# kornia/kornia

Hardware: AMD Instinct MI355X
Metric: Mpix/s fwd+bwd warp_perspective+GaussianBlur2d Bx3x512x512 (higher is better)
Workload: dtype f32; 1 GPU; configs[1]: warp_perspective bilinear + GaussianBlur2d k=5 sigma=1.5, B=256x3x512x512 fp32 fwd+bwd (grad wrt image and homography) per GPU; global_batch=256, parallelism=batch-shard x1 (weak scaling), no data-path collective

## Files before the change

kornia_amd/csrc/km_blur_fast.hip:

```cpp
#include <stdlib.h>

#include "km_regtile.h"


#ifdef KMB_ROWS_OVERRIDE
#define KMB_ROWS KMB_ROWS_OVERRIDE
#else
#define KMB_ROWS 32
#endif
#define KMB_ROWS_MID 16
#define KMB_ROWS_SMALL 8
#define KMB_FEW_WAVES_F32 4096

template <typename T>
struct KmVec4;
template <>
struct KmVec4<float> {
    typedef float4 V;
};
template <>
struct KmVec4<km_bf16> {
    typedef uint2 V;
};
template <>
struct KmVec4<km_f16> {
    typedef uint2 V;
};

__device__ __forceinline__ float km_round_store(float v, const float*) { return v; }
__device__ __forceinline__ float km_round_store(float v, const km_bf16*) { return __uint_as_float(((uint32_t)km_f32_to_bf16_bits(v)) << 16); }
__device__ __forceinline__ float km_round_store(float v, const km_f16*) { KM_OPAQUE(v); return (float)(_Float16)v; }


template <typename T>
struct KmBlurArgs {
    const T* x;
    T* y;
    const float* kx;
    const float* ky;
    int C, H, W, Bk, border;
    uint32_t groups_x;
    uint32_t bx, by;
    uint32_t nblocks;
    uint32_t reverse;
    uint32_t rows;
    uint32_t stream_out;
};

template <int K>
__device__ __forceinline__ void kmb_adjoint_taps(const float (&k)[K], int p, int n, int border, float (&w)[K]) {
    constexpr int L = (K - 1) / 2, R = K - 1 - L;
    const bool interior = (border == KM_BORDER_CIRCULAR) || (border == KM_BORDER_CONSTANT) || (p >= K - 1 && p <= n - K);
#pragma unroll
    for (int d = 0; d < K; ++d) w[d] = k[K - 1 - d];
    if (interior) return;
#pragma unroll
    for (int d = 0; d < K; ++d) {
        const int i = p - R + d;
        float acc = 0.f;
        if (i >= 0 && i < n) {
#pragma unroll
            for (int t = 0; t < K; ++t)
                if (km_border_map(i + t - L, n, border) == p) acc += k[t];
        }
        w[d] = acc;
    }
}

#ifndef KMB_BWD_WAVES
#define KMB_BWD_WAVES 1
#endif
template <typename T, int K, bool BWD, int ROWS = KMB_ROWS>
__global__ __launch_bounds__(256, (BWD ? KMB_BWD_WAVES : 1)) void km_blur_reg_kernel(const KmBlurArgs<T> a) {
    constexpr int L = (K - 1) / 2, R = K - 1 - L;
    constexpr bool COLF = BWD && sizeof(T) == 2;
    uint32_t bid = km_xcd_remap(blockIdx.x, a.nblocks, a.reverse);
    const uint32_t tbx = bid % a.bx;
    bid /= a.bx;
    const uint32_t tby = bid % a.by;
    const uint32_t bc = bid / a.by;
    const int lane = threadIdx.x & 63, wave = __builtin_amdgcn_readfirstlane((int)(threadIdx.x >> 6));
    const int gx = (int)tbx * 64 + lane;
    const int r0 = ((int)tby * 4 + wave) * ROWS;
    if (gx >= (int)a.groups_x || r0 >= a.H) return;
    const int H = a.H, W = a.W, border = a.border;
    const int c0 = gx * 4;
    const bool left = (c0 == 0), right = (c0 == W - 4);
    const T* img = a.x + (size_t)bc * H * W;
    T* out = a.y + (size_t)bc * H * W;
    const int b = (int)(bc / a.C);

    float kx[K], ky[K];
    {
        const float* px = a.kx + (size_t)(b % a.Bk) * K;
        const float* py = a.ky + (size_t)(b % a.Bk) * K;
#pragma unroll
        for (int t = 0; t < K; ++t) { kx[t] = px[t]; ky[t] = py[t]; }
    }
    float wx[4][K];
    if (BWD) {
#pragma unroll
        for (int o = 0; o < 4; ++o) kmb_adjoint_taps<K>(kx, c0 + o, W, border, wx[o]);
    }

    int offL = c0 - 4, offR = c0 + 4;
    if (left) offL = (border == KM_BORDER_CIRCULAR) ? W - 4 : c0;
    if (right) offR = (border == KM_BORDER_CIRCULAR) ? 0 : c0;

    float ring[K][4];
    float ring_e[COLF ? K : 1][COLF ? R : 1];
    const int n_rows = (r0 + ROWS <= H ? ROWS : H - r0);
    const int total = n_rows + K - 1;
    const bool e0 = (lane == 0), e63 = (lane == 63);

    float on4[4] = {0.f, 0.f, 0.f, 0.f}, en4[4] = {0.f, 0.f, 0.f, 0.f};
    int srow_n = -1;
    auto request = [&](int it) {
        const int rin = r0 + it - (BWD ? R : L);
        int sr;
        if (BWD) sr = (border == KM_BORDER_CIRCULAR) ? km_border_map(rin, H, KM_BORDER_CIRCULAR) : ((rin >= 0 && rin < H) ? rin : -1);
        else sr = km_border_map(rin, H, border);
        srow_n = sr;
        if (sr >= 0) {
            const T* rowp = img + (size_t)sr * W;
            km_ld4(rowp + c0, on4);
            if (border != KM_BORDER_CIRCULAR && (e0 || e63)) km_ld4(rowp + (e0 ? offL : offR), en4);
        }
    };
    request(0);

    for (int it0 = 0; it0 < total; it0 += K) {
#pragma unroll
        for (int kk = 0; kk < K; ++kk) {
            const int it = it0 + kk;
            if (it < total) {
                const int srow = srow_n;
                float v[12];
                float o4[4], e4[4];
#pragma unroll
                for (int q = 0; q < 4; ++q) { o4[q] = on4[q]; e4[q] = en4[q]; }
                if (it + 1 < total) request(it + 1);
                if (srow >= 0) {
                    const T* rowp = img + (size_t)srow * W;
                    float l4[4], r4[4];
                    if (border == KM_BORDER_CIRCULAR) {
                        km_ld4(rowp + offL, l4);
                        km_ld4(rowp + offR, r4);
                    } else {
#pragma unroll
                        for (int q = 0; q < 4; ++q) {
                            const float pl = km_prev64(o4[q]), nr = km_next64(o4[q]);
                            l4[q] = e0 ? e4[q] : pl;
                            r4[q] = e63 ? e4[q] : nr;
                        }
                    }
                    if (border != KM_BORDER_CIRCULAR) {
                        if (BWD || border == KM_BORDER_CONSTANT) {
                            if (left) { l4[0] = l4[1] = l4[2] = l4[3] = 0.f; }
                            if (right) { r4[0] = r4[1] = r4[2] = r4[3] = 0.f; }
                        } else if (border == KM_BORDER_REFLECT) {
                            if (left) { l4[0] = r4[0]; l4[1] = o4[3]; l4[2] = o4[2]; l4[3] = o4[1]; }
                            if (right) { const float t3 = l4[3]; r4[0] = o4[2]; r4[1] = o4[1]; r4[2] = o4[0]; r4[3] = t3; }
                        } else {
                            if (left) { l4[0] = l4[1] = l4[2] = l4[3] = o4[0]; }
                            if (right) { r4[0] = r4[1] = r4[2] = r4[3] = o4[3]; }
                        }
                    }
#pragma unroll
                    for (int q = 0; q < 4; ++q) { v[q] = l4[q]; v[4 + q] = o4[q]; v[8 + q] = r4[q]; }
                } else {
#pragma unroll
                    for (int q = 0; q < 12; ++q) v[q] = 0.f;
                }
                if constexpr (COLF) {
#pragma unroll
                    for (int o = 0; o < 4; ++o) ring[kk][o] = v[4 + o];
#pragma unroll
                    for (int j = 0; j < R; ++j) ring_e[kk][j] = e0 ? v[4 - R + j] : v[8 + j];
                } else {
#pragma unroll
                    for (int o = 0; o < 4; ++o) {
                        float acc = 0.f;
                        if (BWD) {
#pragma unroll
                            for (int d = 0; d < K; ++d) acc = km_fma(wx[o][d], v[4 + o - R + d], acc);
                        } else {
#pragma unroll
                            for (int q = 0; q < K; ++q) acc = km_fma(kx[q], v[4 + o - L + q], acc);
                        }
                        ring[kk][o] = km_round_store(acc, (const T*)nullptr);
                    }
                }
                if (it >= K - 1) {
                    const int r = r0 + it - (K - 1);
                    float res[4];
                    if constexpr (COLF) {
                        float wy[K];
                        kmb_adjoint_taps<K>(ky, r, H, border, wy);
                        float c4[4], ce[R];
#pragma unroll
                        for (int o = 0; o < 4; ++o) {
                            float acc = 0.f;
#pragma unroll
                            for (int d = 0; d < K; ++d) acc = km_fma(wy[d], ring[(kk + 1 + d) % K][o], acc);
                            c4[o] = km_round_store(acc, (const T*)nullptr);
                        }
#pragma unroll
                        for (int j = 0; j < R; ++j) {
                            float acc = 0.f;
#pragma unroll
                            for (int d = 0; d < K; ++d) acc = km_fma(wy[d], ring_e[(kk + 1 + d) % K][j], acc);
                            ce[j] = km_round_store(acc, (const T*)nullptr);
                        }
                        float u[12];
#pragma unroll
                        for (int q = 0; q < 4; ++q) {
                            const float pl = km_prev64(c4[q]), nr = km_next64(c4[q]);
                            u[q] = left ? 0.f : pl;
                            u[4 + q] = c4[q];
                            u[8 + q] = right ? 0.f : nr;
                        }
#pragma unroll
                        for (int j = 0; j < R; ++j) {
                            if (e0 && !left) u[4 - R + j] = ce[j];
                            if (e63 && !right) u[8 + j] = ce[j];
                        }
#pragma unroll
                        for (int o = 0; o < 4; ++o) {
                            float acc = 0.f;
#pragma unroll
                            for (int d = 0; d < K; ++d) acc = km_fma(wx[o][d], u[4 + o - R + d], acc);
                            res[o] = acc;
                        }
                    } else if (BWD) {
                        float wy[K];
                        kmb_adjoint_taps<K>(ky, r, H, border, wy);
#pragma unroll
                        for (int o = 0; o < 4; ++o) {
                            float acc = 0.f;
#pragma unroll
                            for (int d = 0; d < K; ++d) acc = km_fma(wy[d], ring[(kk + 1 + d) % K][o], acc);
                            res[o] = acc;
                        }
                    } else {
#pragma unroll
                        for (int o = 0; o < 4; ++o) {
                            float acc = 0.f;
#pragma unroll
                            for (int p = 0; p < K; ++p) acc = km_fma(ky[p], ring[(kk + 1 + p) % K][o], acc);
                            res[o] = acc;
                        }
                    }
                    km_st4_pol(out + (size_t)r * W + c0, res, a.stream_out != 0u);
                }
            }
        }
    }
}

template <typename T, int K, int ROWS>
static void km_blur_launch_rows(bool bwd, const KmBlurArgs<T>& a, hipStream_t s) {
    if (bwd)
        hipLaunchKernelGGL((km_blur_reg_kernel<T, K, true, ROWS>), dim3(a.nblocks), dim3(256), 0, s, a);
    else
        hipLaunchKernelGGL((km_blur_reg_kernel<T, K, false, ROWS>), dim3(a.nblocks), dim3(256), 0, s, a);
}
template <typename T, int K>
static int km_blur_launch(bool bwd, const KmBlurArgs<T>& a, hipStream_t s) {
    if (a.rows == KMB_ROWS_SMALL) km_blur_launch_rows<T, K, KMB_ROWS_SMALL>(bwd, a, s);
    else if (a.rows == KMB_ROWS_MID) km_blur_launch_rows<T, K, KMB_ROWS_MID>(bwd, a, s);
    else km_blur_launch_rows<T, K, KMB_ROWS>(bwd, a, s);
    return km_check_launch(bwd ? "km_blur_reg_bwd" : "km_blur_reg_fwd");
}

static int km_blur_rows(bool bwd, size_t elem, int K, uint64_t waves_big, int force) {
    if (force == KMB_ROWS_SMALL || force == KMB_ROWS_MID || force == KMB_ROWS) return force;
    if (elem == 2) return KMB_ROWS;
    if (waves_big < KMB_FEW_WAVES_F32 || K == 3) return KMB_ROWS_MID;
    if (K == 5) return bwd ? KMB_ROWS : KMB_ROWS_MID;
    return KMB_ROWS;
}

template <typename T>
static int km_blur_run(bool bwd, const void* x, const void* kx, const void* ky, void* y, int B, int C, int H, int W, int Bk,
                       int K, int border, hipStream_t s) {
    KmBlurArgs<T> a;
    a.x = (const T*)x; a.y = (T*)y; a.kx = (const float*)kx; a.ky = (const float*)ky;
    a.C = C; a.H = H; a.W = W; a.Bk = Bk; a.border = border;
    a.groups_x = (uint32_t)(W / 4);
    a.bx = (a.groups_x + 63) / 64;
    const int force_rows = km_config().blur_rows;
    const uint64_t waves_big = (uint64_t)a.bx * (uint64_t)((H + KMB_ROWS - 1) / KMB_ROWS) * (uint64_t)B * C;
    const int rows = km_blur_rows(bwd, sizeof(T), K, waves_big, force_rows);
    a.rows = (uint32_t)rows;
    a.by = (uint32_t)((H + 4 * rows - 1) / (4 * rows));
    const uint64_t nb = (uint64_t)a.bx * a.by * (uint64_t)B * C;
    KM_REQUIRE(nb < (1ull << 31), "km_blur: grid too large");
    a.nblocks = (uint32_t)nb;
    if (nb == 0) return 0;
    a.reverse = km_traversal_next(s);
    a.stream_out = km_stream_stores((uint64_t)B * C * H * W * sizeof(T));
    switch (K) {
        case 3: return km_blur_launch<T, 3>(bwd, a, s);
        case 5: return km_blur_launch<T, 5>(bwd, a, s);
        case 7: return km_blur_launch<T, 7>(bwd, a, s);
        default: return km_blur_launch<T, 9>(bwd, a, s);
    }
}

int km_blur_fast_supported(const void* x, const void* y, int H, int W, int kH, int kW, int border, int same, int dtype) {
    if (!same || kH != kW || (kH & 1) == 0 || kH < 3 || kH > 9) return 0;
    if (dtype == KM_F64) return 0;
    if ((W & 3) != 0 || W < 8 || H < kH) return 0;
    if (border == KM_BORDER_REFLECT && (kH - 1) / 2 >= (H < W ? H : W)) return 0;
    const size_t esz = (dtype == KM_F32) ? 4 : 2;
    if (((uintptr_t)x % (4 * esz)) != 0 || ((uintptr_t)y % (4 * esz)) != 0) return 0;
    if ((((size_t)H * W * esz) % (4 * esz)) != 0) return 0;
    return 1;
}

int km_blur_fast_bwd_supported(const void* gy, const void* gx, int H, int W, int kH, int kW, int border, int same, int dtype) {
    if (dtype != KM_F32 && border == KM_BORDER_CIRCULAR) return 0;
    return km_blur_fast_supported(gy, gx, H, W, kH, kW, border, same, dtype);
}

int km_blur_fast_run(bool bwd, const void* x, const void* kx, const void* ky, void* y, int B, int C, int H, int W, int Bk, int K,
                     int border, int dtype, hipStream_t s) {
    switch (dtype) {
        case KM_F32: return km_blur_run<float>(bwd, x, kx, ky, y, B, C, H, W, Bk, K, border, s);
        case KM_BF16: return km_blur_run<km_bf16>(bwd, x, kx, ky, y, B, C, H, W, Bk, K, border, s);
        default: return km_blur_run<km_f16>(bwd, x, kx, ky, y, B, C, H, W, Bk, K, border, s);
    }
}
```

kornia_amd/csrc/km_common.h:

```cpp
#pragma once

#include <hip/hip_runtime.h>
#include <stdint.h>

#define KM_ABI_FEATURES 3
#define KM_ABI_VERSION 3

enum { KM_F32 = 0, KM_F64 = 1, KM_BF16 = 2, KM_F16 = 3 };

void km_set_error(const char* fmt, ...);
int km_check_launch(const char* what);

#define KM_REQUIRE(cond, ...)          \
    do {                               \
        if (!(cond)) {                 \
            km_set_error(__VA_ARGS__); \
            return -1;                 \
        }                              \
    } while (0)

#ifndef KM_CHECK_ALIGNED
#define KM_CHECK_ALIGNED(p, bytes) ((void)0)
#endif

#ifndef KM_F2I
#define KM_F2I(v) ((int)(v))
#endif

#ifndef KM_CVT_RPI
__device__ __forceinline__ int km_cvt_rpi(float v) {
    int r;
    asm("v_cvt_rpi_i32_f32 %0, %1" : "=v"(r) : "v"(v));
    return r;
}
#define KM_CVT_RPI(v) km_cvt_rpi(v)
#endif

#ifndef KM_NEXT16
__device__ __forceinline__ uint32_t km_next16(uint32_t v) {
    return (uint32_t)__builtin_amdgcn_update_dpp((int)v, (int)v, 0x101, 0xf, 0xf, false);
}
__device__ __forceinline__ float km_next16(float v) { return __uint_as_float(km_next16(__float_as_uint(v))); }
__device__ __forceinline__ float km_prev16(float v) {
    return __uint_as_float((uint32_t)__builtin_amdgcn_update_dpp((int)__float_as_uint(v), (int)__float_as_uint(v), 0x111, 0xf, 0xf, false));
}
__device__ __forceinline__ uint32_t km_next64(uint32_t v) { return (uint32_t)__builtin_amdgcn_update_dpp((int)v, (int)v, 0x130, 0xf, 0xf, false); }
__device__ __forceinline__ float km_next64(float v) { return __uint_as_float(km_next64(__float_as_uint(v))); }
__device__ __forceinline__ float km_prev64(float v) {
    return __uint_as_float((uint32_t)__builtin_amdgcn_update_dpp((int)__float_as_uint(v), (int)__float_as_uint(v), 0x138, 0xf, 0xf, false));
}
__device__ __forceinline__ float km_quad_xor1(float v) {
    return __uint_as_float((uint32_t)__builtin_amdgcn_update_dpp((int)__float_as_uint(v), (int)__float_as_uint(v), 0xB1, 0xf, 0xf, false));
}
__device__ __forceinline__ float km_quad_xor2(float v) {
    return __uint_as_float((uint32_t)__builtin_amdgcn_update_dpp((int)__float_as_uint(v), (int)__float_as_uint(v), 0x4E, 0xf, 0xf, false));
}
__device__ __forceinline__ uint32_t km_wave_umax_last(uint32_t v) {
    int x = (int)v;
#define KM_UMAX_STEP(ctrl, rows) x = (int)max((uint32_t)x, (uint32_t)__builtin_amdgcn_update_dpp(x, x, ctrl, rows, 0xf, false));
    KM_UMAX_STEP(0x111, 0xf) KM_UMAX_STEP(0x112, 0xf) KM_UMAX_STEP(0x114, 0xf) KM_UMAX_STEP(0x118, 0xf)
    KM_UMAX_STEP(0x142, 0xa) KM_UMAX_STEP(0x143, 0xc)
#undef KM_UMAX_STEP
    return (uint32_t)x;
}
__device__ __forceinline__ double km_wave_sum_last(double v) {
#define KM_DSUM_STEP(ctrl, rows)                                                                                  \
    {                                                                                                             \
        const int lo_ = __builtin_amdgcn_update_dpp(0, __double2loint(v), ctrl, rows, 0xf, false);                \
        const int hi_ = __builtin_amdgcn_update_dpp(0, __double2hiint(v), ctrl, rows, 0xf, false);                \
        v += __hiloint2double(hi_, lo_);                                                                          \
    }
    KM_DSUM_STEP(0x111, 0xf) KM_DSUM_STEP(0x112, 0xf) KM_DSUM_STEP(0x114, 0xf) KM_DSUM_STEP(0x118, 0xf)
    KM_DSUM_STEP(0x142, 0xa) KM_DSUM_STEP(0x143, 0xc)
#undef KM_DSUM_STEP
    return v;
}
#endif

__device__ __forceinline__ void km_quad_transpose4(float (&a)[4], int q) {
    const bool b0 = (q & 1) != 0, b1 = (q & 2) != 0;
#pragma unroll
    for (int p = 0; p < 4; p += 2) {
        const float r = km_quad_xor1(b0 ? a[p] : a[p + 1]);
        a[p] = b0 ? r : a[p];
        a[p + 1] = b0 ? a[p + 1] : r;
    }
#pragma unroll
    for (int p = 0; p < 2; ++p) {
        const float r = km_quad_xor2(b1 ? a[p] : a[p + 2]);
        a[p] = b1 ? r : a[p];
        a[p + 2] = b1 ? a[p + 2] : r;
    }
}
template <bool STREAM>
__device__ __forceinline__ void km_st4_c(float* p, const float (&v)[4]) {
    typedef float km_f4v_ __attribute__((ext_vector_type(4)));
    km_f4v_ vv; vv.x = v[0]; vv.y = v[1]; vv.z = v[2]; vv.w = v[3];
    if constexpr (STREAM) __builtin_nontemporal_store(vv, reinterpret_cast<km_f4v_*>(p));
    else *reinterpret_cast<km_f4v_*>(p) = vv;
}

struct km_bf16 {
    uint16_t bits;
};
typedef _Float16 km_f16;

template <typename T>
struct KmTraits;
template <>
struct KmTraits<float> {
    typedef float R;
    static constexpr int code = KM_F32;
};
template <>
struct KmTraits<double> {
    typedef double R;
    static constexpr int code = KM_F64;
};
template <>
struct KmTraits<km_bf16> {
    typedef float R;
    static constexpr int code = KM_BF16;
};
template <>
struct KmTraits<km_f16> {
    typedef float R;
    static constexpr int code = KM_F16;
};

__device__ __forceinline__ float km_ld(const float* p) { return *p; }
__device__ __forceinline__ double km_ld(const double* p) { return *p; }
__device__ __forceinline__ float km_ld(const km_bf16* p) { return __uint_as_float(((uint32_t)p->bits) << 16); }
__device__ __forceinline__ float km_ld(const km_f16* p) { return (float)(*p); }

__device__ __forceinline__ uint16_t km_f32_to_bf16_bits_sw(float f) {
    uint32_t u = __float_as_uint(f);
    if ((u & 0x7fffffffu) > 0x7f800000u) return (uint16_t)((u >> 16) | 0x0040u);
    u += 0x7fffu + ((u >> 16) & 1u);
    return (uint16_t)(u >> 16);
}
#if defined(__gfx950__)
__device__ __forceinline__ uint16_t km_f32_to_bf16_bits(float f) { return __builtin_bit_cast(uint16_t, (__bf16)f); }
__device__ __forceinline__ uint32_t km_f32x2_to_bf16x2_bits(float lo, float hi) {
    typedef __bf16 km_bf2v __attribute__((ext_vector_type(2)));
    typedef float km_f2v_ __attribute__((ext_vector_type(2)));
    km_f2v_ v; v.x = lo; v.y = hi;
    return __builtin_bit_cast(uint32_t, __builtin_convertvector(v, km_bf2v));
}
#else
__device__ __forceinline__ uint16_t km_f32_to_bf16_bits(float f) { return km_f32_to_bf16_bits_sw(f); }
__device__ __forceinline__ uint32_t km_f32x2_to_bf16x2_bits(float lo, float hi) {
    return (uint32_t)km_f32_to_bf16_bits_sw(lo) | ((uint32_t)km_f32_to_bf16_bits_sw(hi) << 16);
}
#endif
#ifndef KM_OPAQUE
#define KM_OPAQUE(v) asm volatile("" : "+v"(v))
#endif
#ifndef KM_NO_NT_ST
#define KM_NT_ST 1
#endif
#ifdef KM_NT_ST
__device__ __forceinline__ void km_st(float* p, float v) { __builtin_nontemporal_store(v, p); }
#else
__device__ __forceinline__ void km_st(float* p, float v) { *p = v; }
#endif
#define KM_STREAM_MIN_BYTES (128ull << 20)
static inline uint32_t km_stream_stores(uint64_t out_bytes) {
#ifdef KM_NT_ST
    return out_bytes >= KM_STREAM_MIN_BYTES ? 1u : 0u;
#else
    (void)out_bytes;
    return 0u;
#endif
}
#ifndef KM_FWD_PLAIN_ST
#define KM_FWD_PLAIN_ST 0
#endif
template <bool STREAM>
__device__ __forceinline__ void km_st_c(float* p, float v) {
    if constexpr (STREAM && !KM_FWD_PLAIN_ST) __builtin_nontemporal_store(v, p);
    else *p = v;
}
__device__ __forceinline__ void km_st(double* p, double v) { *p = v; }
__device__ __forceinline__ void km_st(km_bf16* p, float v) { p->bits = km_f32_to_bf16_bits(v); }
__device__ __forceinline__ void km_st(km_f16* p, float v) { KM_OPAQUE(v); *p = (km_f16)v; }
template <bool STREAM>
__device__ __forceinline__ void km_st_c(double* p, double v) { *p = v; }
template <bool STREAM>
__device__ __forceinline__ void km_st_c(km_bf16* p, float v) { km_st(p, v); }
template <bool STREAM>
__device__ __forceinline__ void km_st_c(km_f16* p, float v) { km_st(p, v); }

__device__ __forceinline__ float km_round_as(float v, const float*) { return v; }
__device__ __forceinline__ double km_round_as(double v, const double*) { return v; }
__device__ __forceinline__ float km_round_as(float v, const km_bf16*) { return __uint_as_float(((uint32_t)km_f32_to_bf16_bits(v)) << 16); }
__device__ __forceinline__ float km_round_as(float v, const km_f16*) { KM_OPAQUE(v); return (float)(km_f16)v; }

struct __attribute__((packed, aligned(4))) km_f32x2_u { float x, y; };
struct __attribute__((packed, aligned(8))) km_f64x2_u { double x, y; };
struct __attribute__((packed, aligned(2))) km_u16x2_u { uint16_t x, y; };
__device__ __forceinline__ void km_ld2(const float* p, float& a, float& b) {
    const km_f32x2_u v = *reinterpret_cast<const km_f32x2_u*>(p);
    a = v.x; b = v.y;
}
__device__ __forceinline__ void km_ld2(const double* p, double& a, double& b) {
    const km_f64x2_u v = *reinterpret_cast<const km_f64x2_u*>(p);
    a = v.x; b = v.y;
}
__device__ __forceinline__ void km_ld2(const km_bf16* p, float& a, float& b) {
    const km_u16x2_u v = *reinterpret_cast<const km_u16x2_u*>(p);
    a = __uint_as_float(((uint32_t)v.x) << 16); b = __uint_as_float(((uint32_t)v.y) << 16);
}
struct __attribute__((packed, aligned(2))) km_h16x2_u { km_f16 x, y; };
__device__ __forceinline__ void km_ld2(const km_f16* p, float& a, float& b) {
    const km_h16x2_u v = *reinterpret_cast<const km_h16x2_u*>(p);
    a = (float)v.x; b = (float)v.y;
}

struct __attribute__((packed, aligned(4))) km_f32x4_u { float x, y, z, w; };
struct __attribute__((packed, aligned(8))) km_f64x4_u { double x, y, z, w; };
struct __attribute__((packed, aligned(2))) km_u16x4_u { uint16_t x, y, z, w; };
__device__ __forceinline__ void km_ld4u(const float* p, float (&o)[4]) {
    const km_f32x4_u v = *reinterpret_cast<const km_f32x4_u*>(p);
    o[0] = v.x; o[1] = v.y; o[2] = v.z; o[3] = v.w;
}
__device__ __forceinline__ void km_ld4u(const double* p, double (&o)[4]) {
    const km_f64x4_u v = *reinterpret_cast<const km_f64x4_u*>(p);
    o[0] = v.x; o[1] = v.y; o[2] = v.z; o[3] = v.w;
}
__device__ __forceinline__ void km_ld4u(const km_bf16* p, float (&o)[4]) {
    const km_u16x4_u v = *reinterpret_cast<const km_u16x4_u*>(p);
    o[0] = __uint_as_float(((uint32_t)v.x) << 16); o[1] = __uint_as_float(((uint32_t)v.y) << 16);
    o[2] = __uint_as_float(((uint32_t)v.z) << 16); o[3] = __uint_as_float(((uint32_t)v.w) << 16);
}
__device__ __forceinline__ void km_ld4u(const km_f16* p, float (&o)[4]) {
    o[0] = (float)p[0]; o[1] = (float)p[1]; o[2] = (float)p[2]; o[3] = (float)p[3];
}

template <typename T>
__device__ __forceinline__ const T* km_at(const T* base, uint32_t elem_off) {
    return reinterpret_cast<const T*>(reinterpret_cast<const char*>(base) + elem_off * (uint32_t)sizeof(T));
}

template <typename T>
__device__ __forceinline__ T* km_at_mut(T* base, uint32_t elem_off) {
    return reinterpret_cast<T*>(reinterpret_cast<char*>(base) + elem_off * (uint32_t)sizeof(T));
}

__device__ __host__ __forceinline__ float km_fma(float a, float b, float c) { return __builtin_fmaf(a, b, c); }
__device__ __host__ __forceinline__ double km_fma(double a, double b, double c) { return __builtin_fma(a, b, c); }
__device__ __forceinline__ float km_floor(float x) { return __builtin_floorf(x); }
__device__ __forceinline__ double km_floor(double x) { return __builtin_floor(x); }
__device__ __forceinline__ float km_fabs(float x) { return __builtin_fabsf(x); }
__device__ __forceinline__ double km_fabs(double x) { return __builtin_fabs(x); }
__device__ __forceinline__ float km_rint(float x) { return __builtin_rintf(x); }
__device__ __forceinline__ double km_rint(double x) { return __builtin_rint(x); }
__device__ __forceinline__ float km_fmod(float a, float b) { return fmodf(a, b); }
__device__ __forceinline__ double km_fmod(double a, double b) { return fmod(a, b); }
__device__ __forceinline__ float km_sqrt(float x) { return __builtin_sqrtf(x); }
__device__ __forceinline__ double km_sqrt(double x) { return __builtin_sqrt(x); }

__device__ __forceinline__ void km_atomic_add(float* p, float v) { unsafeAtomicAdd(p, v); }
__device__ __forceinline__ void km_atomic_add(double* p, double v) { unsafeAtomicAdd(p, v); }

__device__ __forceinline__ uint32_t km_xcd_remap(uint32_t bid, uint32_t nblocks, uint32_t reverse = 0u) {
    const uint32_t NX = 8;
    const uint32_t q = nblocks / NX, r = nblocks % NX;
    const uint32_t xcd = bid % NX, k = bid / NX;
    const uint32_t start = xcd * q + (xcd < r ? xcd : r);
    const uint32_t count = q + (xcd < r ? 1u : 0u);
    return start + (reverse ? count - 1u - k : k);
}

#ifndef KM_GLDS16
__device__ __forceinline__ uint32_t km_lds_addr(const void* p) {
    return (uint32_t)__builtin_amdgcn_readfirstlane((int)(uint32_t)(uintptr_t)(const __attribute__((address_space(3))) char*)p);
}
__device__ __forceinline__ void km_glds16(const void* gsrc, uint32_t lds_dst) {
    uint32_t keep;
    asm volatile("s_mov_b32 %0, m0\n\ts_mov_b32 m0, %2\n\ts_nop 0\n\tglobal_load_lds_dwordx4 %1, off\n\ts_mov_b32 m0, %0" : "=&s"(keep) : "v"(gsrc), "s"(lds_dst) : "memory");
}
__device__ __forceinline__ void km_glds4(const void* gsrc, uint32_t lds_dst) {
    uint32_t keep;
    asm volatile("s_mov_b32 %0, m0\n\ts_mov_b32 m0, %2\n\ts_nop 0\n\tglobal_load_lds_dword %1, off\n\ts_mov_b32 m0, %0" : "=&s"(keep) : "v"(gsrc), "s"(lds_dst) : "memory");
}
#define KM_GLDS16(gsrc, lds_wave_base) km_glds16((const void*)(gsrc), km_lds_addr(lds_wave_base))
#define KM_GLDS4(gsrc, lds_wave_base) km_glds4((const void*)(gsrc), km_lds_addr(lds_wave_base))
#define KM_VMCNT0() asm volatile("s_waitcnt vmcnt(0)" ::: "memory")
#endif

#ifndef KM_TID_PINNED
__device__ __forceinline__ int km_tid_pinned() {
    int t = (int)threadIdx.x;
#ifndef KM_TID_UNPINNED
    asm volatile("" : "+v"(t));
#endif
    return t;
}
#endif

#ifndef KM_SCHED_FENCE
#define KM_SCHED_FENCE() __builtin_amdgcn_sched_barrier(0)
#endif

uint32_t km_traversal_next(hipStream_t s);

#ifndef KM_PAIR_FUSED_DEFAULT
#define KM_PAIR_FUSED_DEFAULT 2
#endif
struct KmConfig {
    int traversal_fixed;
    int warp_fwd_algo;
    int warp_gm_algo;
    int warp_bwd_generic;
    int warp_bwd_fused;
    int sep_lds;
    int sg_generic;
    int pyrdown_separable;
    int blur_rows;
    int pair_fused;
    int warp_bwd_no_scan;
};
const KmConfig& km_config();
int km_device_cus();
hipStream_t km_side_fork(hipStream_t s);
int km_side_join(hipStream_t s);

#ifndef KM_LDS_BARRIER
#define KM_LDS_BARRIER() asm volatile("s_waitcnt lgkmcnt(0)\n\ts_barrier" ::: "memory")
#endif

__device__ __forceinline__ double km_wave_sum(double v) {
#pragma unroll
    for (int off = 32; off > 0; off >>= 1) v += __shfl_down(v, off, 64);
    return v;
}
```

Before: 47650 Mpix/s.

## Batch blur halo-column loads into per-wave gathers read via readlane

Replaces the per-row edge loads by lanes 0 and 63 with a batched gather. Lanes 0-31 fetch the left halo and lanes 32-63 fetch the right halo for up to 32 rows at once, and each row reads its value back with readlane. Out-of-range lanes now stay alive, clamped and masked on store, so the whole wave can take part in the gather. This removes divergent single-lane loads from the per-row critical path. In exchange it adds readlane instructions and a second gather when the row count exceeds 32.

```diff
diff --git a/kornia_amd/csrc/km_blur_fast.hip b/kornia_amd/csrc/km_blur_fast.hip
--- a/kornia_amd/csrc/km_blur_fast.hip
+++ b/kornia_amd/csrc/km_blur_fast.hip
@@ -80,9 +80,10 @@
     const uint32_t tby = bid % a.by;
     const uint32_t bc = bid / a.by;
     const int lane = threadIdx.x & 63, wave = __builtin_amdgcn_readfirstlane((int)(threadIdx.x >> 6));
-    const int gx = (int)tbx * 64 + lane;
     const int r0 = ((int)tby * 4 + wave) * ROWS;
-    if (gx >= (int)a.groups_x || r0 >= a.H) return;
+    if (r0 >= a.H) return;
+    const bool live = (int)tbx * 64 + lane < (int)a.groups_x;
+    const int gx = live ? (int)tbx * 64 + lane : (int)a.groups_x - 1;
     const int H = a.H, W = a.W, border = a.border;
     const int c0 = gx * 4;
     const bool left = (c0 == 0), right = (c0 == W - 4);
@@ -113,32 +114,48 @@
     const int total = n_rows + K - 1;
     const bool e0 = (lane == 0), e63 = (lane == 63);
 
-    float on4[4] = {0.f, 0.f, 0.f, 0.f}, en4[4] = {0.f, 0.f, 0.f, 0.f};
+    float on4[4] = {0.f, 0.f, 0.f, 0.f};
     int srow_n = -1;
+    auto source_row = [&](int it) {
+        const int rin = r0 + it - (BWD ? R : L);
+        if (BWD) return (border == KM_BORDER_CIRCULAR) ? km_border_map(rin, H, KM_BORDER_CIRCULAR) : ((rin >= 0 && rin < H) ? rin : -1);
+        return km_border_map(rin, H, border);
+    };
     auto request = [&](int it) {
-        const int rin = r0 + it - (BWD ? R : L);
-        int sr;
-        if (BWD) sr = (border == KM_BORDER_CIRCULAR) ? km_border_map(rin, H, KM_BORDER_CIRCULAR) : ((rin >= 0 && rin < H) ? rin : -1);
-        else sr = km_border_map(rin, H, border);
+        const int sr = source_row(it);
         srow_n = sr;
-        if (sr >= 0) {
-            const T* rowp = img + (size_t)sr * W;
-            km_ld4(rowp + c0, on4);
-            if (border != KM_BORDER_CIRCULAR && (e0 || e63)) km_ld4(rowp + (e0 ? offL : offR), en4);
+        if (sr >= 0 && live) km_ld4(img + (size_t)sr * W + c0, on4);
+    };
+    constexpr bool TWO_GATHERS = (ROWS + K - 1 > 32);
+    float g4[4] = {0.f, 0.f, 0.f, 0.f};
+    const bool need_l = (tbx != 0u), need_r = ((int)tbx * 256 + 256 < W);
+    const bool gathers = (border != KM_BORDER_CIRCULAR) && (need_l || need_r);
+    auto gather = [&](int base) {
+        int gl = lane;
+        KM_OPAQUE(gl);
+        const bool side_r = (gl >= 32);
+        const int gc = side_r ? (int)tbx * 256 + 256 : (int)tbx * 256 - 4;
+        const bool need = side_r ? need_r : need_l;
+        const int gi = base + (gl & 31);
+        const int sr = source_row(gi);
+        if (need && gi < total && sr >= 0) km_ld4(img + (size_t)sr * W + gc, g4);
+    };
+    if (gathers) gather(0);
+    request(0);
+
+    for (int it0 = 0; it0 < total; it0 += K) {
+        if constexpr (TWO_GATHERS) {
+            if (gathers && total > 32 && it0 + 2 * K >= 32 && it0 + K < 32) gather(32);
         }
-    };
-    request(0);
-
-    for (int it0 = 0; it0 < total; it0 += K) {
 #pragma unroll
         for (int kk = 0; kk < K; ++kk) {
             const int it = it0 + kk;
             if (it < total) {
                 const int srow = srow_n;
                 float v[12];
-                float o4[4], e4[4];
-#pragma unroll
-                for (int q = 0; q < 4; ++q) { o4[q] = on4[q]; e4[q] = en4[q]; }
+                float o4[4];
+#pragma unroll
+                for (int q = 0; q < 4; ++q) o4[q] = on4[q];
                 if (it + 1 < total) request(it + 1);
                 if (srow >= 0) {
                     const T* rowp = img + (size_t)srow * W;
@@ -147,11 +164,13 @@
                         km_ld4(rowp + offL, l4);
                         km_ld4(rowp + offR, r4);
                     } else {
+                        const int gl = it & 31;
 #pragma unroll
                         for (int q = 0; q < 4; ++q) {
                             const float pl = km_prev64(o4[q]), nr = km_next64(o4[q]);
-                            l4[q] = e0 ? e4[q] : pl;
-                            r4[q] = e63 ? e4[q] : nr;
+                            const float el = km_readlane(g4[q], gl), er = km_readlane(g4[q], 32 + gl);
+                            l4[q] = e0 ? el : pl;
+                            r4[q] = e63 ? er : nr;
                         }
                     }
                     if (border != KM_BORDER_CIRCULAR) {
@@ -251,7 +270,7 @@
                             res[o] = acc;
                         }
                     }
-                    km_st4_pol(out + (size_t)r * W + c0, res, a.stream_out != 0u);
+                    if (live) km_st4_pol(out + (size_t)r * W + c0, res, a.stream_out != 0u);
                 }
             }
         }
diff --git a/kornia_amd/csrc/km_common.h b/kornia_amd/csrc/km_common.h
--- a/kornia_amd/csrc/km_common.h
+++ b/kornia_amd/csrc/km_common.h
@@ -75,6 +75,11 @@
 #undef KM_DSUM_STEP
     return v;
 }
+__device__ __forceinline__ float km_readlane(float v, int src) {
+    return __uint_as_float((uint32_t)__builtin_amdgcn_readlane((int)__float_as_uint(v), src));
+}
+#else
+__device__ __forceinline__ float km_readlane(float v, int src) { return __shfl(v, src, 64); }
 #endif
 
 __device__ __forceinline__ void km_quad_transpose4(float (&a)[4], int q) {
```

Measured after the change: 47620 Mpix/s. Within noise of the previous version (-0.1%).
